# chaoting-sun/GCT-Plus

Measured on AMD Instinct MI355X. Metric: SMILES/sec training step (vaetf, seq_len=80, d_model=512), higher is better.
Workload: dtype f32

## Files before the change

### gct_plus_amd/csrc/norm.hip

```cpp
#include "common.h"

namespace {

constexpr int MAXC = 8;

template <int NC>
__global__ __launch_bounds__(256) void norm_fwd_kernel(const float* __restrict__ x,
                                                       const float* __restrict__ alpha,
                                                       const float* __restrict__ bias, float* y,
                                                       float* mean_out, float* rstd_out,
                                                       int64_t rows, int d, float eps) {
  const int lane = threadIdx.x & 63, wave = threadIdx.x >> 6;
  const int64_t nwaves = (int64_t)gridDim.x * 4;
  float4 a[NC], b[NC];
#pragma unroll
  for (int c = 0; c < NC; ++c) {
    const int col = c * 256 + lane * 4;
    if (col < d) {
      a[c] = *reinterpret_cast<const float4*>(alpha + col);
      b[c] = *reinterpret_cast<const float4*>(bias + col);
    }
  }
  for (int64_t row = (int64_t)blockIdx.x * 4 + wave; row < rows; row += nwaves) {
    const float* xr = x + row * d;
    float4 v[NC];
    float s = 0.f;
#pragma unroll
    for (int c = 0; c < NC; ++c) {
      const int col = c * 256 + lane * 4;
      v[c] = make_float4(0.f, 0.f, 0.f, 0.f);
      if (col < d) {
        v[c] = *reinterpret_cast<const float4*>(xr + col);
        s += (v[c].x + v[c].y) + (v[c].z + v[c].w);
      }
    }
    const float mean = gct_wave_sum(s) / (float)d;
    float ss = 0.f;
#pragma unroll
    for (int c = 0; c < NC; ++c) {
      const int col = c * 256 + lane * 4;
      if (col < d) {
        v[c].x -= mean; v[c].y -= mean; v[c].z -= mean; v[c].w -= mean;
        ss += (v[c].x * v[c].x + v[c].y * v[c].y) + (v[c].z * v[c].z + v[c].w * v[c].w);
      }
    }
    const float var = gct_wave_sum(ss) / (float)(d - 1);
    const float rstd = 1.0f / (sqrtf(var) + eps);
    if (lane == 0) {
      mean_out[row] = mean;
      rstd_out[row] = rstd;
    }
    float* yr = y + row * d;
#pragma unroll
    for (int c = 0; c < NC; ++c) {
      const int col = c * 256 + lane * 4;
      if (col < d) {
        float4 o;
        o.x = a[c].x * (v[c].x * rstd) + b[c].x;
        o.y = a[c].y * (v[c].y * rstd) + b[c].y;
        o.z = a[c].z * (v[c].z * rstd) + b[c].z;
        o.w = a[c].w * (v[c].w * rstd) + b[c].w;
        *reinterpret_cast<float4*>(yr + col) = o;
      }
    }
  }
}

template <int NC>
__global__ __launch_bounds__(256) void norm_bwd_kernel(const float* __restrict__ dy,
                                                       const float* __restrict__ x,
                                                       const float* __restrict__ alpha,
                                                       const float* __restrict__ mean_in,
                                                       const float* __restrict__ rstd_in,
                                                       const float* __restrict__ dres, float* dx,
                                                       float* partial, int64_t rows, int d,
                                                       float eps, const int32_t* __restrict__ qmap,
                                                       int64_t src_rows, float* dropo, uint32_t thr, float dscale,
                                                       GctRng rng) {
  const int lane = threadIdx.x & 63, wave = threadIdx.x >> 6;
  const int64_t nwaves = (int64_t)gridDim.x * 4;
  float4 a[NC], pa[NC], pb[NC];
#pragma unroll
  for (int c = 0; c < NC; ++c) {
    const int col = c * 256 + lane * 4;
    a[c] = make_float4(0.f, 0.f, 0.f, 0.f);
    if (col < d) a[c] = *reinterpret_cast<const float4*>(alpha + col);
    pa[c] = make_float4(0.f, 0.f, 0.f, 0.f);
    pb[c] = make_float4(0.f, 0.f, 0.f, 0.f);
  }
  const int64_t nquads = (rows + 3) >> 2;
  for (int64_t quad = (int64_t)blockIdx.x * 4 + wave; quad < nquads; quad += nwaves) {
   uint4 db[NC][2];
   if (dropo) {
     const int64_t oq = qmap ? (int64_t)qmap[quad] : quad;
#pragma unroll
     for (int c = 0; c < NC; ++c) {
       const int col = c * 256 + lane * 4;
       db[c][0] = gct_drop_bits(rng, (uint32_t)(oq < 0 ? 0 : oq), (uint32_t)col);
       db[c][1] = gct_drop_bits(rng, (uint32_t)(oq < 0 ? 0 : oq), (uint32_t)col + 2);
     }
   }
   for (int e4 = 0; e4 < 4; ++e4) {
    const int64_t row = quad * 4 + e4;
    if (row >= rows) break;
    int64_t srow = row;
    if (qmap) {
      const int q = qmap[row >> 2];
      if (src_rows > 0) srow = (int64_t)q * 4 + (row & 3);
      if (q < 0 || (src_rows > 0 && srow >= src_rows)) {
        float* dr0 = dx + row * d;
#pragma unroll
        for (int c = 0; c < NC; ++c) {
          const int col = c * 256 + lane * 4;
          if (col < d) {
            *reinterpret_cast<float4*>(dr0 + col) = make_float4(0.f, 0.f, 0.f, 0.f);
            if (dropo) *reinterpret_cast<float4*>(dropo + row * d + col) = make_float4(0.f, 0.f, 0.f, 0.f);
          }
        }
        continue;
      }
    }
    const float mean = mean_in[srow], r = rstd_in[srow];
    const float* xr = x + srow * d;
    const float* gr = dy + row * d;
    float4 cx[NC], g[NC];
    float s1 = 0.f, s2 = 0.f;
#pragma unroll
    for (int c = 0; c < NC; ++c) {
      const int col = c * 256 + lane * 4;
      cx[c] = make_float4(0.f, 0.f, 0.f, 0.f);
      g[c] = cx[c];
      if (col < d) {
        float4 xv = *reinterpret_cast<const float4*>(xr + col);
        const float4 dv = *reinterpret_cast<const float4*>(gr + col);
        xv.x -= mean; xv.y -= mean; xv.z -= mean; xv.w -= mean;
        cx[c] = xv;
        pa[c].x += dv.x * xv.x * r; pa[c].y += dv.y * xv.y * r;
        pa[c].z += dv.z * xv.z * r; pa[c].w += dv.w * xv.w * r;
        pb[c].x += dv.x; pb[c].y += dv.y; pb[c].z += dv.z; pb[c].w += dv.w;
        g[c] = make_float4(dv.x * a[c].x, dv.y * a[c].y, dv.z * a[c].z, dv.w * a[c].w);
        s1 += (g[c].x + g[c].y) + (g[c].z + g[c].w);
        s2 += (g[c].x * xv.x + g[c].y * xv.y) + (g[c].z * xv.z + g[c].w * xv.w);
      }
    }
    s1 = gct_wave_sum(s1) / (float)d;
    s2 = gct_wave_sum(s2);
    const float sigma = 1.0f / r - eps;
    const float k2 = sigma > 0.f ? s2 * r * r / (sigma * (float)(d - 1)) : 0.f;
    float* dr = dx + row * d;
#pragma unroll
    for (int c = 0; c < NC; ++c) {
      const int col = c * 256 + lane * 4;
      if (col < d) {
        float4 o;
        o.x = r * (g[c].x - s1) - cx[c].x * k2;
        o.y = r * (g[c].y - s1) - cx[c].y * k2;
        o.z = r * (g[c].z - s1) - cx[c].z * k2;
        o.w = r * (g[c].w - s1) - cx[c].w * k2;
        if (dres) {
          const float4 e = *reinterpret_cast<const float4*>(dres + row * d + col);
          o.x += e.x; o.y += e.y; o.z += e.z; o.w += e.w;
        }
        *reinterpret_cast<float4*>(dr + col) = o;
        if (dropo) {
          const int e = e4;
          const uint4 b0 = db[c][0], b1 = db[c][1];
          float4 m;
// ... 9 lines not shown
  }
  __shared__ float4 comb[4][64];
#pragma unroll
  for (int c = 0; c < NC; ++c) {
    const int col = c * 256 + lane * 4;
    for (int which = 0; which < 2; ++which) {
      __syncthreads();
      comb[wave][lane] = which == 0 ? pa[c] : pb[c];
      __syncthreads();
      if (wave == 0 && col < d) {
        float4 t = comb[0][lane];
        for (int w = 1; w < 4; ++w) {
          t.x += comb[w][lane].x; t.y += comb[w][lane].y;
          t.z += comb[w][lane].z; t.w += comb[w][lane].w;
        }
        *reinterpret_cast<float4*>(partial + ((int64_t)blockIdx.x * 2 + which) * d + col) = t;
      }
    }
  }
}

inline int norm_blocks(int64_t rows) {
  int64_t b = (rows + 3) / 4;
  if (b > 1024) b = 1024;
  if (b < 1) b = 1;
  return (int)b;
}

}

int gct_reduce_slabs_seg(const float* slabs, int nslab, int64_t stride, float* d0, float* d1,
                         float* d2, int64_t nper_elems, int64_t n, hipStream_t st);

#define NORM_DISPATCH(KERNEL, ...)                                                      \
  do {                                                                                  \
    const int nc = (d + 255) / 256;                                                     \
    if (nc <= 1) hipLaunchKernelGGL((KERNEL<1>), grid, dim3(256), 0, st, __VA_ARGS__);  \
    else if (nc <= 2) hipLaunchKernelGGL((KERNEL<2>), grid, dim3(256), 0, st, __VA_ARGS__); \
    else if (nc <= 4) hipLaunchKernelGGL((KERNEL<4>), grid, dim3(256), 0, st, __VA_ARGS__); \
    else hipLaunchKernelGGL((KERNEL<8>), grid, dim3(256), 0, st, __VA_ARGS__);          \
  } while (0)

extern "C" int gct_norm_fwd(const float* x, const float* alpha, const float* bias, float* y,
                            float* mean, float* rstd, int64_t rows, int d, float eps,
                            void* stream) {
  GCT_CHECK_ARG(x && alpha && bias && y && mean && rstd, "norm_fwd: null pointer");
  GCT_CHECK_ARG(rows >= 0 && d >= 4 && d % 4 == 0 && d <= 256 * MAXC, "norm_fwd: d=%d unsupported", d);
  GCT_CHECK_ARG(gct_aligned16(x) && gct_aligned16(y) && gct_aligned16(alpha) && gct_aligned16(bias),
                "norm_fwd: pointers must be 16-B aligned");
  if (rows == 0) return GCT_OK;
  hipStream_t st = (hipStream_t)stream;
  dim3 grid((unsigned)((rows + 3) / 4 > 8192 ? 8192 : (rows + 3) / 4));
  NORM_DISPATCH(norm_fwd_kernel, x, alpha, bias, y, mean, rstd, rows, d, eps);
  GCT_LAUNCH_CHECK("norm_fwd");
  return GCT_OK;
}

extern "C" int gct_norm_bwd(const float* dy, const float* x, const float* alpha, const float* mean,
                            const float* rstd, const float* dres, float* dx, float* dalpha,
                            float* dbias, float* ws, int64_t rows, int d, float eps,
                            const int32_t* quad_map, int64_t src_rows, float* drop_out, float p, uint64_t seed,
                            uint32_t site, void* stream) {
  GCT_CHECK_ARG(dy && x && alpha && mean && rstd && dx && dalpha && dbias && ws,
                "norm_bwd: null pointer");
  GCT_CHECK_ARG(!drop_out || (gct_aligned16(drop_out) && p >= 0.f && p < 1.f), "norm_bwd: bad dropout output");
  GCT_CHECK_ARG(!quad_map || (rows % 4 == 0 && src_rows >= 0), "norm_bwd: compacted rows come in quads");
  GCT_CHECK_ARG(rows >= 0 && d >= 4 && d % 4 == 0 && d <= 256 * MAXC, "norm_bwd: d=%d unsupported", d);
  GCT_CHECK_ARG(gct_aligned16(dy) && gct_aligned16(x) && gct_aligned16(dx) && gct_aligned16(alpha) &&
                    gct_aligned16(ws) && (!dres || gct_aligned16(dres)),
                "norm_bwd: pointers must be 16-B aligned");
  hipStream_t st = (hipStream_t)stream;
  const int nblk = norm_blocks(rows);
  dim3 grid((unsigned)nblk);
  NORM_DISPATCH(norm_bwd_kernel, dy, x, alpha, mean, rstd, dres, dx, ws, rows, d, eps, quad_map, src_rows, drop_out,
                gct_drop_threshold(p), 1.0f / (1.0f - p), gct_rng_make(seed, site));
  GCT_LAUNCH_CHECK("norm_bwd");
  return gct_reduce_slabs_seg(ws, nblk, (int64_t)2 * d, dalpha, dbias, nullptr, d, (int64_t)2 * d, st);
}
```

### gct_plus_amd/engine.py

```python
from __future__ import annotations

import math
import os
from typing import List, NamedTuple, Optional

import torch
from torch.autograd.function import once_differentiable

from . import ops
from .flat import HANDED_SLOTS

_SEED = {"base": None, "ctr": 0}

COMPACT_BWD = os.environ.get("GCT_COMPACT_BWD", "1") != "0"
COMPACT_MAX_FRACTION = 0.85
COMPACT_KV = os.environ.get("GCT_COMPACT_KV", "1") != "0"
COMPACT_FWD = os.environ.get("GCT_COMPACT_FWD", "1") != "0"
COMPACT_ENC_KV = os.environ.get("GCT_COMPACT_ENC_KV", "1") != "0"
KV_FOLD = True


GRAD_NOTIFY = None


# ... 210 lines not shown
class EncoderSaved(NamedTuple):
    src: torch.Tensor
    econds: Optional[torch.Tensor]
    site_pe: int
    layers: List[EncLayerSaved]
    x_last: torch.Tensor
    mean: torch.Tensor
    rstd: torch.Tensor
    B: int
    L: int


class DecoderSaved(NamedTuple):
    trg: torch.Tensor
    z2: torch.Tensor
    dconds: Optional[torch.Tensor]
    site_pe: int
    layers: List[DecLayerSaved]
    x_last: torch.Tensor
    mean: torch.Tensor
    rstd: torch.Tensor
    B: int
    T: int
    Le: int
    Lk: int
    c2d: bool
    c2l: bool
    trg_mask_u8: Optional[torch.Tensor]
    keys: object
    live: object
    fold: object = None


def mha_fwd(run: Run, m, xq, xkv, B, Lq, Lk, mask_u8, resid, want_probs=False, keys=None, live=None, fold=None):
    d, H = m.d_model, m.h
    dk = d // H
    self_attn = xkv is xq
    Mq = xq.shape[0]
    self_split = self_attn and keys is not None and live is None and not want_probs
    if self_split:
        xkv = keys.gather(xq)
    if self_attn and not self_split:
        qkv = _empty(Mq, 3 * d, xq)
        ops.linear_fwd(xq, [m.q_linear.weight, m.k_linear.weight, m.v_linear.weight],
                       [m.q_linear.bias, m.k_linear.bias, m.v_linear.bias],
                       [qkv, qkv[:, d:], qkv[:, 2 * d:]], 3 * d)
        q, k, v, ldq, ldkv = qkv, qkv[:, d:], qkv[:, 2 * d:], 3 * d, 3 * d
        qb, kvb = qkv, None
        if live is not None:
            keys = live
    else:
        qb = _empty(Mq, d, xq)
        ops.linear_fwd(xq, [m.q_linear.weight], [m.q_linear.bias], [qb], d)
        kvb = _empty(B * Lk, 2 * d, xkv) if keys is None else keys.empty(2 * d)
        if fold is not None:
            fold[0].fwd(fold[1], xkv, [kvb, kvb[:, d:]], 2 * d)
        else:
            ops.linear_fwd(xkv, [m.k_linear.weight, m.v_linear.weight],
                           [m.k_linear.bias, m.v_linear.bias], [kvb, kvb[:, d:]], 2 * d)
        q, k, v, ldq, ldkv = qb, kvb, kvb[:, d:], d, 2 * d
    site_p = run.site()
    o, lse, probs = ops.attn_fwd(q, k, v, ldq, ldkv, ldkv, mask_u8, B, H, Lq, Lk, dk, run.p,
                                 run.seed, site_p, want_probs=want_probs, keys=keys, live=live)
    y = _empty(Mq, d, xq)
    site_o = run.site()
    if resid is not None:
        ops.linear_fwd(o, [m.out.weight], [m.out.bias], [y], d, epi=ops.EPI_DROP_RESID,
                       resid=resid, p=run.p, seed=run.seed, site=site_o, live=live)
    else:
        ops.linear_fwd(o, [m.out.weight], [m.out.bias], [y], d)
    saved = MhaSaved(xq, xkv, qb, kvb, o, lse, mask_u8, B, Lq, Lk, site_p, site_o, resid is not None,
                     None if (self_attn and live is not None) else keys, self_split)
    return y, saved, probs


def mha_bwd(run: Run, m, sv: MhaSaved, dy, G: GradSink, dxq_out, depi_q, dxkv_out=None,
            depi_kv=ops.DEPI_STORE, live=None, gdrop=None, fold=None):
    B, Lq, Lk, keys = sv.B, sv.Lq, sv.Lk, sv.keys
    d, H = m.d_model, m.h
    dk = d // H
    Mq, Mk = B * Lq, sv.xkv.shape[0]
    kt = run.kt
    new = lambda cols: _empty(Mq, cols, dy)
    if live is not None:
        Mq, kt = live.Mc, None
        new = live.empty_zero_gaps
        o_in, xq_in = (sv.o, sv.xq) if live.fwd else (live.gather(sv.o), live.gather(sv.xq))
    else:
        o_in, xq_in = sv.o, sv.xq
    if gdrop is not None:
        g = gdrop
    else:
        g = ops.dropout_bwd(dy, run.p, run.seed, sv.site_o, live=live) if (sv.fused and run.p > 0) else dy
    do = _empty(Mq, d, dy) if live is None else live.empty(d)
    ops.linear_bwd([g], d, o_in, [m.out.weight], [G(m.out.weight)], [G(m.out.bias)], do, kt=kt, M=Mq)
    if sv.kvb is None:
        dqkv = new(3 * d)
        fwdc = live is not None and live.fwd
        ops.attn_bwd(sv.qb, sv.qb[:, d:], sv.qb[:, 2 * d:], 3 * d, 3 * d, 3 * d, sv.mask_u8, sv.o, do, sv.lse, dqkv,
                     dqkv[:, d:], dqkv[:, 2 * d:], 3 * d, 3 * d, 3 * d, B, H, Lq, Lk, dk, run.p,
                     run.seed, sv.site_p, live=live, kv_compact=live is not None and not fwdc,
                     keys=live if fwdc else None)
        segs = [dqkv, dqkv[:, d:], dqkv[:, 2 * d:]]
        ops.linear_bwd(segs, 3 * d, xq_in, [m.q_linear.weight, m.k_linear.weight, m.v_linear.weight],
                       [G(m.q_linear.weight), G(m.k_linear.weight), G(m.v_linear.weight)],
                       [G(m.q_linear.bias), G(m.k_linear.bias), G(m.v_linear.bias)], dxq_out, depi=depi_q, kt=kt, M=Mq)
    else:
        dq = new(d)
        if keys is None:
            dkv = _empty(Mk, 2 * d, dy)
        else:
            dkv = keys.empty_zero_gaps(2 * d)
        ops.attn_bwd(sv.qb, sv.kvb, sv.kvb[:, d:], d, 2 * d, 2 * d, sv.mask_u8, sv.o, do, sv.lse, dq, dkv, dkv[:, d:],
                     d, 2 * d, 2 * d, B, H, Lq, Lk, dk, run.p, run.seed, sv.site_p, live=live, keys=keys)
        ops.linear_bwd([dq], d, xq_in, [m.q_linear.weight], [G(m.q_linear.weight)], [G(m.q_linear.bias)], dxq_out,
                       depi=depi_q, kt=kt, M=Mq)
        if fold is not None:
            fold[0].bwd(fold[1], [dkv, dkv[:, d:]], 2 * d, sv.xkv, dxkv_out, depi_kv, Mk)
            return
        kv_w = [m.k_linear.weight, m.v_linear.weight]
        kv_g = ([G(m.k_linear.weight), G(m.v_linear.weight)], [G(m.k_linear.bias), G(m.v_linear.bias)])
        if sv.self_split:
            dxk = keys.empty(d)
            ops.linear_bwd([dkv, dkv[:, d:]], 2 * d, sv.xkv, kv_w, *kv_g, dxk, M=Mk)
            keys.scatter_add(dxk, dxq_out)
        elif dxkv_out is not None:
            ops.linear_bwd([dkv, dkv[:, d:]], 2 * d, sv.xkv, kv_w, *kv_g, dxkv_out, depi=depi_kv, M=Mk)
        else:
            ops.linear_wgrad([dkv, dkv[:, d:]], 2 * d, sv.xkv, *kv_g)


def ffn_fwd(run: Run, ff, x, resid, live=None):
    M, d = x.shape
    dff = ff.linear_1.weight.shape[0]
    gelu_d = _empty(M, dff, x)
    hdn = _empty(M, dff, x)
    site_h = run.site()
    ops.linear_fwd(x, [ff.linear_1.weight], [ff.linear_1.bias], [hdn], dff, epi=ops.EPI_GELU_DROP_SAVE,
                   pre=gelu_d, p=run.p, seed=run.seed, site=site_h, live=live)
    y = _empty(M, d, x)
    site_o = run.site()
    if resid is not None:
        ops.linear_fwd(hdn, [ff.linear_2.weight], [ff.linear_2.bias], [y], d,
                       epi=ops.EPI_DROP_RESID, resid=resid, p=run.p, seed=run.seed, site=site_o, live=live)
    else:
        ops.linear_fwd(hdn, [ff.linear_2.weight], [ff.linear_2.bias], [y], d)
    return y, FfnSaved(x, gelu_d, hdn, site_h, site_o, resid is not None)


def ffn_bwd(run: Run, ff, sv: FfnSaved, dy, G: GradSink, dx_out, depi, live=None, gdrop=None):
    x, gelu_d, hdn = sv.x, sv.gelu_d, sv.hdn
    M, d = x.shape
    dff = gelu_d.shape[1]
    kt = run.kt
    if live is not None:
        M, kt = live.Mc, None
        if not live.fwd:
            x, hdn = live.gather(x), live.gather(hdn)
    if gdrop is not None:
        g = gdrop
    else:
        g = ops.dropout_bwd(dy, run.p, run.seed, sv.site_o, live=live) if (sv.fused and run.p > 0) else dy
    dpre = _empty(M, dff, dy) if live is None else live.empty(dff)
    ops.linear_bwd([g], d, hdn, [ff.linear_2.weight], [G(ff.linear_2.weight)], [G(ff.linear_2.bias)], dpre,
                   depi=ops.DEPI_MUL_SAVED, pre=gelu_d, p=run.p, seed=run.seed, site=sv.site_h, kt=kt, live=live,
                   pre_full=live is not None and not live.fwd, M=M)
    ops.linear_bwd([dpre], dff, x, [ff.linear_1.weight], [G(ff.linear_1.weight)], [G(ff.linear_1.bias)], dx_out,
                   depi=depi, kt=kt, M=M)


def enc_layer_fwd(run: Run, layer, x_in, B, L, mask_u8, want_probs=False, keys=None):
    n1, m1, r1 = ops.norm_fwd(x_in, layer.norm_1.alpha, layer.norm_1.bias, layer.norm_1.eps)
    a, sv_a, probs = mha_fwd(run, layer.attn, n1, n1, B, L, L, mask_u8, n1, want_probs, keys=keys)
    n2, m2, r2 = ops.norm_fwd(a, layer.norm_2.alpha, layer.norm_2.bias, layer.norm_2.eps)
    out, sv_f = ffn_fwd(run, layer.ff, n2, n2)
    return out, EncLayerSaved(x_in, m1, r1, sv_a, a, m2, r2, sv_f), probs


def _mha_drop(run: Run, sv: MhaSaved, buf):
    return (buf, run.p, run.seed, sv.site_o) if (buf is not None and sv.fused and run.p > 0) else None


def _ffn_drop(run: Run, sv: Optional[FfnSaved], buf):
    return (buf, run.p, run.seed, sv.site_o) if (buf is not None and sv is not None and sv.fused and run.p > 0) else None


def enc_layer_bwd(run: Run, layer, sv: EncLayerSaved, g, G: GradSink, gd=None, gdbuf=None, below=None):
    with ops.deferred_reductions():
        ffn_bwd(run, layer.ff, sv.ffn, g, G, g, ops.DEPI_ACCUM, gdrop=gd)
        dr = _mha_drop(run, sv.attn, gdbuf)
        ops.norm_bwd(g, sv.a, layer.norm_2.alpha, sv.m2, sv.r2, G(layer.norm_2.alpha), G(layer.norm_2.bias),
                     out=g, eps=layer.norm_2.eps, drop=dr)
        mha_bwd(run, layer.attn, sv.attn, g, G, g, ops.DEPI_ACCUM, gdrop=None if dr is None else gdbuf)
        dr = _ffn_drop(run, below, gdbuf)
        ops.norm_bwd(g, sv.x_in, layer.norm_1.alpha, sv.m1, sv.r1, G(layer.norm_1.alpha), G(layer.norm_1.bias),
                     out=g, eps=layer.norm_1.eps, drop=dr)
    _grads_done(layer, G)
    return g, (None if dr is None else gdbuf)


def dec_layer_fwd(run: Run, layer, x, e, B, T, Lk, src_mask_u8, trg_mask_u8, want_probs=False, keys=None, live=None,
                  fold=None):
    x2, m1, r1 = ops.norm_fwd(x, layer.norm_1.alpha, layer.norm_1.bias, layer.norm_1.eps)
    xa, sa1, p1 = mha_fwd(run, layer.attn_1, x2, x2, B, T, T, trg_mask_u8, x, want_probs, live=live)
    x2, m2, r2 = ops.norm_fwd(xa, layer.norm_2.alpha, layer.norm_2.bias, layer.norm_2.eps)
    xb, sa2, p2 = mha_fwd(run, layer.attn_2, x2, e, B, T, Lk, src_mask_u8, xa, want_probs, keys=keys, live=live,
                          fold=fold)
    x2, m3, r3 = ops.norm_fwd(xb, layer.norm_3.alpha, layer.norm_3.bias, layer.norm_3.eps)
    xc, sf = ffn_fwd(run, layer.ff, x2, xb, live=live)
    return xc, DecLayerSaved(x, m1, r1, sa1, xa, m2, r2, sa2, xb, m3, r3, sf), p1, p2


def dec_layer_bwd(run: Run, layer, sv: DecLayerSaved, g, de, first_de, G: GradSink, live=None, gd=None, gdbuf=None,
                  below=None, fold=None):
    t = torch.empty_like(g) if live is None else live.empty(g.shape[1])
    with ops.deferred_reductions():
        ffn_bwd(run, layer.ff, sv.ffn, g, G, t, ops.DEPI_STORE, live=live, gdrop=gd)
        dr = _mha_drop(run, sv.attn_2, gdbuf)
        ops.norm_bwd(t, sv.xb, layer.norm_3.alpha, sv.m3, sv.r3, G(layer.norm_3.alpha), G(layer.norm_3.bias),
                     dres=g, out=g, eps=layer.norm_3.eps, live=live, drop=dr)
        mha_bwd(run, layer.attn_2, sv.attn_2, g, G, t, ops.DEPI_STORE, de,
                ops.DEPI_STORE if first_de else ops.DEPI_ACCUM, live=live, gdrop=None if dr is None else gdbuf,
                fold=fold)
        dr = _mha_drop(run, sv.attn_1, gdbuf)
        ops.norm_bwd(t, sv.xa, layer.norm_2.alpha, sv.m2, sv.r2, G(layer.norm_2.alpha), G(layer.norm_2.bias),
                     dres=g, out=g, eps=layer.norm_2.eps, live=live, drop=dr)
        mha_bwd(run, layer.attn_1, sv.attn_1, g, G, t, ops.DEPI_STORE, live=live, gdrop=None if dr is None else gdbuf)
        dr = _ffn_drop(run, below, gdbuf)
        ops.norm_bwd(t, sv.x, layer.norm_1.alpha, sv.m1, sv.r1, G(layer.norm_1.alpha), G(layer.norm_1.bias),
# ... 608 lines not shown
```

### gct_plus_amd/ops.py

```python
from __future__ import annotations

import contextlib
import math
import os
import threading
import weakref
from typing import List, Optional, Sequence

import torch

from . import _lib
from ._lib import check

EPI_BIAS, EPI_GELU_DROP, EPI_DROP_RESID, EPI_GELU_DROP_SAVE = 0, 1, 2, 3
DEPI_STORE, DEPI_ACCUM, DEPI_GELU_BWD, DEPI_MUL_SAVED = 0, 1, 2, 3


def _L():
    return _lib.load()


_raw_stream, _cur_dev = torch._C._cuda_getCurrentRawStream, torch._C._cuda_getDevice


# ... 98 lines not shown

    def __exit__(self, et, ev, tb):
        if self.mine:
            _DEFER_TL.d["on"] = False
            _DEFER_TL.d["want"] = max(_DEFER_TL.d["want"], _DEFER_TL.d["demand"])
            rc = _L().gct_reduce_defer_end(_st())
            if et is None:
                check(rc, "gct_reduce_defer_end")
        return False


_WS_NEED = {}


def _ws_need(fn: str, a: int, b: int, c: int) -> int:
    key = (fn, a, b, c)
    v = _WS_NEED.get(key)
    if v is None:
        v = _WS_NEED[key] = int(getattr(_L(), fn)(a, b, c))
    return v


def norm_fwd(x2d, alpha, bias, eps=1e-6, out=None):
    _chk(x2d, "norm_fwd.x")
    rows, d = x2d.shape
    y = torch.empty_like(x2d) if out is None else out
    mean = torch.empty(rows, dtype=torch.float32, device=x2d.device)
    rstd = torch.empty(rows, dtype=torch.float32, device=x2d.device)
    check(_L().gct_norm_fwd(_p(x2d), _p(alpha), _p(bias), _p(y), _p(mean), _p(rstd), rows, d, eps,
                            _st()), "gct_norm_fwd")
    return y, mean, rstd


def norm_bwd(dy, x2d, alpha, mean, rstd, dalpha, dbias, dres=None, out=None, eps=1e-6, live=None, drop=None):
    src_rows, d = x2d.shape
    rows = src_rows if live is None else live.Mc
    if live is not None and live.fwd:
        src_rows = 0
    dx = (torch.empty_like(x2d) if live is None else live.empty(d)) if out is None else out
    _wait_pending(out)
    if drop is not None:
        _wait_pending(drop[0])
    ws = kept_workspace(_L().gct_rowred_ws_bytes(rows, 2 * d), x2d.device)
    check(_L().gct_norm_bwd(_p(dy), _p(x2d), _p(alpha), _p(mean), _p(rstd), _p(dres), _p(dx),
                            _p(dalpha), _p(dbias), _p(ws), rows, d, eps,
                            None if live is None else _p(live.quad_list), src_rows,
                            None if drop is None else _p(drop[0]), 0.0 if drop is None else drop[1],
                            0 if drop is None else drop[2], 0 if drop is None else drop[3], _st()), "gct_norm_bwd")
    return dx


def embed_pe_fwd(tok, table, cond, pe2d, n_c, scale, p, seed, site, d=None):
    _chk(tok, "embed.tok", torch.int64)
    B, S = tok.shape
    if table is not None:
        vocab, d = table.shape
    else:
        vocab = 1
    out = torch.empty(B * (S + n_c), d, dtype=torch.float32, device=pe2d.device)
    check(_L().gct_embed_pe_fwd(_p(tok), _p(table), _p(cond), _p(pe2d), _p(out), B, S, n_c, d, vocab,
                                scale, p, seed, site, _st()), "gct_embed_pe_fwd")
    return out


def embed_pe_bwd(dout, tok, dtable, dcond, n_c, scale, p, seed, site, d=None):
    B, S = tok.shape
    if dtable is not None:
        vocab, d = dtable.shape
    else:
        vocab = 1
    ws = kept_workspace(_L().gct_embed_ws_bytes(B, S, d, vocab), dout.device)
    check(_L().gct_embed_pe_bwd(_p(dout), _p(tok), _p(dtable), _p(dcond), _p(ws), B, S, n_c, d, vocab,
                                scale, p, seed, site, _st()), "gct_embed_pe_bwd")


PROFILE = None
PROFILE_KINDS = None


class _Timed:
    def __init__(self, kind, flops, nbytes=0):
# ... 200 lines not shown


def assert_no_skipped_row_gradients():
    n = int(skipped_row_gradients().item())
    if n:
        skipped_row_gradients().zero_()
        raise _lib.GctError(_SKIPPED_MSG.format(n))


def skipped_row_gradients():
    dev = torch.cuda.current_device()
    t = _SKIPPED.get(dev)
    if t is None:
        t = _SKIPPED[dev] = torch.zeros(1, dtype=torch.int32, device=torch.device("cuda", dev))
    return t


class LiveRows:
    SLACK = 256
    fwd = False

    def __init__(self, g2d, B, T, mask_u8, lists=True):
        _chk(g2d, "g2d")
        dev = g2d.device
        M = B * T
        assert g2d.shape[0] == M
        nt, nq = (M + 31) // 32, (M + 3) // 4
        i32 = lambda n: torch.empty(max(n, 1), dtype=torch.int32, device=dev)
        self.B, self.T, self.M, self.dev = B, T, M, dev
        self.live = torch.empty(max(M, 1), dtype=torch.uint8, device=dev)
        self.n_b, self.info = i32(B), i32(8)
        self.cstart = i32(B) if lists else None
        self.quad_list = i32(nq + 32) if lists else None
        qrank = i32(nq) if lists else None
        self.tile_list, self.tile_count = i32(nt), i32(1)
        flags = torch.empty(max(nt, 1), dtype=torch.uint8, device=dev)
        if mask_u8 is None:
            sb = sq = 0
        else:
            _chk(mask_u8, "live_rows.mask", torch.uint8)
            sb, sq = _mask_strides(mask_u8, B, T, T)
        check(_L().gct_live_rows(_p(g2d), g2d.stride(0), B, T, g2d.shape[1], _p(mask_u8), sb, sq, _p(self.live),
                                 _p(self.n_b), _p(self.info), _p(self.cstart), _p(self.quad_list), _p(qrank),
                                 _p(self.tile_list), _p(self.tile_count), _p(flags), _st()), "gct_live_rows")
        self.kt = (self.tile_list, self.tile_count)
        self._host = None
        self.Mc = None

    @classmethod
    def from_rows(cls, rows_u8, B, T, mask_u8):
        _chk(rows_u8, "live_rows.rows", torch.uint8)
        return cls(rows_u8.reshape(B * T, 1).to(torch.float32), B, T, mask_u8)

    def _fill_host(self, v):
        self._host = dict(n_live=v[0], violations=v[1], nonprefix=v[2], tiles=v[3], padded=v[4], quads=v[5], empty=v[6])
        self.Mc = v[4]

    def host(self):
        if self._host is None:
            PendingReadBack(self).finish()
        return self._host

    def scatter_add(self, src2d, dst2d):
        cols = src2d.shape[1]
        check(_L().gct_scatter_add_quads(_p(src2d), src2d.stride(0), _p(self.quad_list), self.Mc, cols, _p(dst2d),
                                         dst2d.stride(0), self.M, _st()), "gct_scatter_add_quads")
        return dst2d

    def check_grad(self, g2d):
        check(_L().gct_dead_rows_nonzero(_p(g2d), g2d.stride(0), self.M, g2d.shape[1], _p(self.live),
                                         _p(skipped_row_gradients()), _st()), "gct_dead_rows_nonzero")

    def empty(self, cols):
        return torch.empty(self.Mc + self.SLACK, cols, dtype=torch.float32, device=self.dev)[:self.Mc]

    def empty_zero_gaps(self, cols):
# ... 35 lines not shown
            self.host.copy_(dev, non_blocking=True)
            self.ev = torch.cuda.Event()
            self.ev.record()

    def finish(self):
        if self.host is None:
            return
        import time
        t0 = time.perf_counter()
        self.ev.synchronize()
        HOST_BLOCKED_S[0] += time.perf_counter() - t0
        v = self.host.tolist()
        self.host = None
        for i, o in enumerate(self.objs):
            if o._host is None:
                o._fill_host(v[8 * i:8 * i + 8])
        if v[-1] != 0:
            skipped_row_gradients().zero_()
            raise _lib.GctError(_SKIPPED_MSG.format(v[-1]))


class KeyRows(LiveRows):

    def __init__(self, mask_u8, B, Lk):
        _chk(mask_u8, "key_rows.mask", torch.uint8)
        dev = mask_u8.device
        M = B * Lk
        nq = (M + 3) // 4
        i32 = lambda n: torch.empty(max(n, 1), dtype=torch.int32, device=dev)
        self.B, self.T, self.M, self.dev = B, Lk, M, dev
        self.live = torch.empty(max(M, 1), dtype=torch.uint8, device=dev)
        self.n_b, self.info = i32(B), i32(8)
        self.cstart, self.quad_list = i32(B), i32(nq + 32)
        qrank = i32(nq)
        check(_L().gct_key_rows(_p(mask_u8), Lk, B, Lk, _p(self.live), _p(self.n_b), _p(self.info), _p(self.cstart),
                                _p(self.quad_list), _p(qrank), _st()), "gct_key_rows")
        self._host = None
        self.Mc = None



def linear_wgrad(dys: Sequence[torch.Tensor], lddy: int, x2d, dws: Sequence[torch.Tensor],
                 dbs: Sequence[Optional[torch.Tensor]], kt=None):
    M, K = x2d.shape
    nper = dws[0].shape[0]
    nseg = len(dws)
    d = _seg3(dys)
    dw = _seg3(dws)
    db = _seg3(dbs)

    def launch():
        ws = kept_workspace(_ws_need("gct_wgrad_ws_bytes", M, nseg * nper, K), x2d.device)
        with _Timed("gemm_wgrad+bias+reduce", 2.0 * M * K * nper * nseg):
            check(_L().gct_linear_wgrad(d[0], d[1], d[2], lddy, M, nseg, nper, _p(x2d), x2d.stride(0),
                                        K, dw[0], dw[1], dw[2], K, db[0], db[1], db[2], _p(ws),
                                        _p(kt[0]) if kt else None, _p(kt[1]) if kt else None, _st()),
                  "gct_linear_wgrad")

    if not SIDE_ENABLED or torch.cuda.is_current_stream_capturing():
        launch()
        return
    main = torch.cuda.current_stream()
    side = _side_stream(x2d.device)
    ready = torch.cuda.Event()
    ready.record(main)
    side.wait_event(ready)
    with torch.cuda.stream(side):
        launch()
        done = torch.cuda.Event()
# ... 841 lines not shown
```

### include/gctplus_hip.h

```cpp
#ifndef GCTPLUS_HIP_H
#define GCTPLUS_HIP_H

#include <stdint.h>

#ifdef __cplusplus
extern "C" {
#endif

#define GCT_OK 0
#define GCT_ERR_ARG (-1)
#define GCT_ERR_HIP (-2)

#define GCT_ABI_VERSION 33

int gct_version(void);
const char* gct_last_error(void);

int64_t gct_wgrad_ws_bytes(int64_t M, int64_t Ntot, int64_t K);
int64_t gct_rowred_ws_bytes(int64_t rows, int64_t cols);

int gct_norm_fwd(const float* x, const float* alpha, const float* bias, float* y,
                 float* mean, float* rstd, int64_t rows, int d, float eps, void* stream);
int gct_norm_bwd(const float* dy, const float* x, const float* alpha, const float* mean,
                 const float* rstd, const float* dres, float* dx, float* dalpha, float* dbias,
                 float* ws, int64_t rows, int d, float eps, const int32_t* quad_map, int64_t src_rows,
                 float* drop_out, float p, uint64_t seed, uint32_t site, void* stream);

int gct_embed_pe_fwd(const int64_t* tok, const float* table, const float* cond, const float* pe,
                     float* out, int B, int S, int n_c, int d, int vocab, float scale, float p,
                     uint64_t seed, uint32_t site, void* stream);
int64_t gct_embed_ws_bytes(int B, int S, int d, int vocab);
int gct_embed_pe_bwd(const float* dout, const int64_t* tok, float* dtable, float* dcond,
                     float* ws, int B, int S, int n_c, int d, int vocab, float scale, float p,
                     uint64_t seed, uint32_t site, void* stream);

#define GCT_EPI_BIAS 0
#define GCT_EPI_GELU_DROP 1
#define GCT_EPI_DROP_RESID 2
#define GCT_EPI_GELU_DROP_SAVE 3
int gct_linear_fwd(const float* x, int64_t ldx, int64_t M, int K,
                   const float* w0, const float* w1, const float* w2, int64_t ldw,
                   const uint16_t* wp0, int64_t plane_stride,
                   const float* b0, const float* b1, const float* b2,
                   int nseg, int nper, float* y0, float* y1, float* y2, int64_t ldy,
                   int epi, const float* resid, float* pre, float p, uint64_t seed, uint32_t site,
                   float* ws, int64_t ws_bytes, const int32_t* quad_map, void* stream);
int64_t gct_linear_fwd_ws_bytes(int64_t M, int K, int Ntot);

#define GCT_DEPI_STORE 0
#define GCT_DEPI_ACCUM 1
#define GCT_DEPI_GELU_BWD 2
#define GCT_DEPI_MUL_SAVED 3
int gct_linear_dgrad(const float* dy0, const float* dy1, const float* dy2, int64_t lddy,
                     int64_t M, int nseg, int nper,
                     const float* w0, const float* w1, const float* w2, int64_t ldw,
                     const uint16_t* wp0, int64_t plane_stride, int K,
                     float* dx, int64_t lddx, int depi, const float* pre, float p, uint64_t seed,
                     uint32_t site, float* ws, int64_t ws_bytes, const int32_t* quad_map, int64_t pre_rows,
                     void* stream);
// ... 298 lines not shown
```

Before: 11770.

## Fuse key-row gather into norm forward and scatter-add into norm backward

The encoder's first layer norm now also writes the compacted live-key rows straight from its forward kernel, so the separate gather launch for self-attention keys/values is no longer needed. In backward, the compact key gradient is added inside the norm backward kernel rather than through a separate scatter-add into the residual gradient. This removes two extra kernel launches and a full read-modify-write pass over the activations per encoder layer. In exchange the norm kernels gain per-quad rank lookups and a tail pass that zero-fills padding rows, and the engine now has more plumbing through the compaction metadata.

```diff
diff --git a/gct_plus_amd/csrc/norm.hip b/gct_plus_amd/csrc/norm.hip
--- a/gct_plus_amd/csrc/norm.hip
+++ b/gct_plus_amd/csrc/norm.hip
@@ -4,12 +4,26 @@
 
 constexpr int MAXC = 8;
 
-template <int NC>
+__device__ __forceinline__ int64_t norm_compact_quad(const int32_t* __restrict__ qrank, const uint8_t* __restrict__ live,
+                                                     int64_t rows, int64_t cquads, int64_t q) {
+  const int64_t qs = __builtin_amdgcn_readfirstlane((int)q);
+  const int64_t rk = qrank[qs];
+  uint32_t f = 0;
+  if (qs * 4 + 4 <= rows) f = *reinterpret_cast<const uint32_t*>(live + qs * 4);
+  else
+    for (int64_t r = qs * 4; r < rows; ++r) f |= live[r];
+  return (f != 0 && rk < cquads) ? rk : -1;
+}
+
+template <int NC, bool COPY>
 __global__ __launch_bounds__(256) void norm_fwd_kernel(const float* __restrict__ x,
                                                        const float* __restrict__ alpha,
                                                        const float* __restrict__ bias, float* y,
                                                        float* mean_out, float* rstd_out,
-                                                       int64_t rows, int d, float eps) {
+                                                       int64_t rows, int d, float eps,
+                                                       const int32_t* __restrict__ qlist,
+                                                       const int32_t* __restrict__ qrank,
+                                                       const uint8_t* __restrict__ live, int64_t cquads, float* yc) {
   const int lane = threadIdx.x & 63, wave = threadIdx.x >> 6;
   const int64_t nwaves = (int64_t)gridDim.x * 4;
   float4 a[NC], b[NC];
@@ -21,8 +35,13 @@
       b[c] = *reinterpret_cast<const float4*>(bias + col);
     }
   }
+  int64_t cq_next = -1;
+  if (COPY && (int64_t)blockIdx.x * 4 + wave < rows)
+    cq_next = norm_compact_quad(qrank, live, rows, cquads, ((int64_t)blockIdx.x * 4 + wave) >> 2);
   for (int64_t row = (int64_t)blockIdx.x * 4 + wave; row < rows; row += nwaves) {
     const float* xr = x + row * d;
+    const int64_t crow = cq_next >= 0 ? cq_next * 4 + (row & 3) : -1;
+    if (COPY && row + nwaves < rows) cq_next = norm_compact_quad(qrank, live, rows, cquads, (row + nwaves) >> 2);
     float4 v[NC];
     float s = 0.f;
 #pragma unroll
@@ -61,12 +80,27 @@
         o.z = a[c].z * (v[c].z * rstd) + b[c].z;
         o.w = a[c].w * (v[c].w * rstd) + b[c].w;
         *reinterpret_cast<float4*>(yr + col) = o;
-      }
-    }
-  }
-}
-
-template <int NC>
+        if (COPY && crow >= 0) *reinterpret_cast<float4*>(yc + crow * d + col) = o;
+      }
+    }
+  }
+  if (COPY) {
+    const float4 z = make_float4(0.f, 0.f, 0.f, 0.f);
+    for (int64_t cq = (int64_t)blockIdx.x * 4 + wave; cq < cquads; cq += nwaves) {
+      const int64_t q = qlist[cq];
+      for (int e = 0; e < 4; ++e)
+        if (q < 0 || q * 4 + e >= rows) {
+#pragma unroll
+          for (int c = 0; c < NC; ++c) {
+            const int col = c * 256 + lane * 4;
+            if (col < d) *reinterpret_cast<float4*>(yc + (cq * 4 + e) * d + col) = z;
+          }
+        }
+    }
+  }
+}
+
+template <int NC, bool ADD>
 __global__ __launch_bounds__(256) void norm_bwd_kernel(const float* __restrict__ dy,
                                                        const float* __restrict__ x,
                                                        const float* __restrict__ alpha,
@@ -76,7 +110,9 @@
                                                        float* partial, int64_t rows, int d,
                                                        float eps, const int32_t* __restrict__ qmap,
                                                        int64_t src_rows, float* dropo, uint32_t thr, float dscale,
-                                                       GctRng rng) {
+                                                       GctRng rng, const float* __restrict__ addc,
+                                                       const int32_t* __restrict__ aqrank,
+                                                       const uint8_t* __restrict__ alive, int64_t acquads) {
   const int lane = threadIdx.x & 63, wave = threadIdx.x >> 6;
   const int64_t nwaves = (int64_t)gridDim.x * 4;
   float4 a[NC], pa[NC], pb[NC];
@@ -89,6 +125,9 @@
     pb[c] = make_float4(0.f, 0.f, 0.f, 0.f);
   }
   const int64_t nquads = (rows + 3) >> 2;
+  int64_t aq_next = -1;
+  if (ADD && (int64_t)blockIdx.x * 4 + wave < nquads)
+    aq_next = norm_compact_quad(aqrank, alive, rows, acquads, (int64_t)blockIdx.x * 4 + wave);
   for (int64_t quad = (int64_t)blockIdx.x * 4 + wave; quad < nquads; quad += nwaves) {
    uint4 db[NC][2];
    if (dropo) {
@@ -100,6 +139,8 @@
        db[c][1] = gct_drop_bits(rng, (uint32_t)(oq < 0 ? 0 : oq), (uint32_t)col + 2);
      }
    }
+   const int64_t arow0 = aq_next >= 0 ? aq_next * 4 : -1;
+   if (ADD && quad + nwaves < nquads) aq_next = norm_compact_quad(aqrank, alive, rows, acquads, quad + nwaves);
    for (int e4 = 0; e4 < 4; ++e4) {
     const int64_t row = quad * 4 + e4;
     if (row >= rows) break;
@@ -132,7 +173,11 @@
       g[c] = cx[c];
       if (col < d) {
         float4 xv = *reinterpret_cast<const float4*>(xr + col);
-        const float4 dv = *reinterpret_cast<const float4*>(gr + col);
+        float4 dv = *reinterpret_cast<const float4*>(gr + col);
+        if (ADD && arow0 >= 0) {
+          const float4 av = *reinterpret_cast<const float4*>(addc + (arow0 + e4) * d + col);
+          dv.x += av.x; dv.y += av.y; dv.z += av.z; dv.w += av.w;
+        }
         xv.x -= mean; xv.y -= mean; xv.z -= mean; xv.w -= mean;
         cx[c] = xv;
         pa[c].x += dv.x * xv.x * r; pa[c].y += dv.y * xv.y * r;
@@ -208,35 +253,58 @@
 int gct_reduce_slabs_seg(const float* slabs, int nslab, int64_t stride, float* d0, float* d1,
                          float* d2, int64_t nper_elems, int64_t n, hipStream_t st);
 
-#define NORM_DISPATCH(KERNEL, ...)                                                      \
-  do {                                                                                  \
-    const int nc = (d + 255) / 256;                                                     \
-    if (nc <= 1) hipLaunchKernelGGL((KERNEL<1>), grid, dim3(256), 0, st, __VA_ARGS__);  \
-    else if (nc <= 2) hipLaunchKernelGGL((KERNEL<2>), grid, dim3(256), 0, st, __VA_ARGS__); \
-    else if (nc <= 4) hipLaunchKernelGGL((KERNEL<4>), grid, dim3(256), 0, st, __VA_ARGS__); \
-    else hipLaunchKernelGGL((KERNEL<8>), grid, dim3(256), 0, st, __VA_ARGS__);          \
+#define NORM_DISPATCH(KERNEL, FLAG, ...)                                                      \
+  do {                                                                                        \
+    const int nc = (d + 255) / 256;                                                           \
+    if (nc <= 1) hipLaunchKernelGGL((KERNEL<1, FLAG>), grid, dim3(256), 0, st, __VA_ARGS__);  \
+    else if (nc <= 2) hipLaunchKernelGGL((KERNEL<2, FLAG>), grid, dim3(256), 0, st, __VA_ARGS__); \
+    else if (nc <= 4) hipLaunchKernelGGL((KERNEL<4, FLAG>), grid, dim3(256), 0, st, __VA_ARGS__); \
+    else hipLaunchKernelGGL((KERNEL<8, FLAG>), grid, dim3(256), 0, st, __VA_ARGS__);          \
   } while (0)
 
-extern "C" int gct_norm_fwd(const float* x, const float* alpha, const float* bias, float* y,
-                            float* mean, float* rstd, int64_t rows, int d, float eps,
-                            void* stream) {
+extern "C" int gct_norm_fwd_rows(const float* x, const float* alpha, const float* bias, float* y, float* mean,
+                                 float* rstd, int64_t rows, int d, float eps, const int32_t* quad_list,
+                                 const int32_t* quad_rank, const uint8_t* live, int64_t crows, float* yc, void* stream) {
   GCT_CHECK_ARG(x && alpha && bias && y && mean && rstd, "norm_fwd: null pointer");
   GCT_CHECK_ARG(rows >= 0 && d >= 4 && d % 4 == 0 && d <= 256 * MAXC, "norm_fwd: d=%d unsupported", d);
   GCT_CHECK_ARG(gct_aligned16(x) && gct_aligned16(y) && gct_aligned16(alpha) && gct_aligned16(bias),
                 "norm_fwd: pointers must be 16-B aligned");
+  GCT_CHECK_ARG((quad_list == nullptr) == (quad_rank == nullptr) && (quad_list == nullptr) == (yc == nullptr) &&
+                    (quad_list == nullptr) == (live == nullptr),
+                "norm_fwd: quad_list / quad_rank / live / yc go together");
+  GCT_CHECK_ARG(!quad_list || (crows >= 0 && crows % 4 == 0 && gct_aligned16(yc) &&
+                               (reinterpret_cast<uintptr_t>(live) & 3u) == 0),
+                "norm_fwd: the compact copy is whole quads of 16-B aligned rows, live is 4-B aligned");
+  hipStream_t st = (hipStream_t)stream;
+  if (quad_list) {
+    if (rows == 0 && crows == 0) return GCT_OK;
+    int64_t work = (rows + 3) / 4 > crows / 16 ? (rows + 3) / 4 : crows / 16;
+    dim3 grid((unsigned)(work > 8192 ? 8192 : (work < 1 ? 1 : work)));
+    NORM_DISPATCH(norm_fwd_kernel, true, x, alpha, bias, y, mean, rstd, rows, d, eps, quad_list, quad_rank, live, crows / 4,
+                  yc);
+    GCT_LAUNCH_CHECK("norm_fwd_rows");
+    return GCT_OK;
+  }
   if (rows == 0) return GCT_OK;
-  hipStream_t st = (hipStream_t)stream;
   dim3 grid((unsigned)((rows + 3) / 4 > 8192 ? 8192 : (rows + 3) / 4));
-  NORM_DISPATCH(norm_fwd_kernel, x, alpha, bias, y, mean, rstd, rows, d, eps);
+  NORM_DISPATCH(norm_fwd_kernel, false, x, alpha, bias, y, mean, rstd, rows, d, eps, (const int32_t*)nullptr,
+                (const int32_t*)nullptr, (const uint8_t*)nullptr, (int64_t)0, (float*)nullptr);
   GCT_LAUNCH_CHECK("norm_fwd");
   return GCT_OK;
 }
 
-extern "C" int gct_norm_bwd(const float* dy, const float* x, const float* alpha, const float* mean,
-                            const float* rstd, const float* dres, float* dx, float* dalpha,
-                            float* dbias, float* ws, int64_t rows, int d, float eps,
-                            const int32_t* quad_map, int64_t src_rows, float* drop_out, float p, uint64_t seed,
-                            uint32_t site, void* stream) {
+extern "C" int gct_norm_fwd(const float* x, const float* alpha, const float* bias, float* y,
+                            float* mean, float* rstd, int64_t rows, int d, float eps,
+                            void* stream) {
+  return gct_norm_fwd_rows(x, alpha, bias, y, mean, rstd, rows, d, eps, nullptr, nullptr, nullptr, 0, nullptr, stream);
+}
+
+extern "C" int gct_norm_bwd_rows(const float* dy, const float* x, const float* alpha, const float* mean,
+                                 const float* rstd, const float* dres, float* dx, float* dalpha, float* dbias, float* ws,
+                                 int64_t rows, int d, float eps, const int32_t* quad_map, int64_t src_rows,
+                                 float* drop_out, float p, uint64_t seed, uint32_t site, const float* add,
+                                 const int32_t* add_quad_rank, const uint8_t* add_live, int64_t add_rows,
+                                 void* stream) {
   GCT_CHECK_ARG(dy && x && alpha && mean && rstd && dx && dalpha && dbias && ws,
                 "norm_bwd: null pointer");
   GCT_CHECK_ARG(!drop_out || (gct_aligned16(drop_out) && p >= 0.f && p < 1.f), "norm_bwd: bad dropout output");
@@ -245,11 +313,32 @@
   GCT_CHECK_ARG(gct_aligned16(dy) && gct_aligned16(x) && gct_aligned16(dx) && gct_aligned16(alpha) &&
                     gct_aligned16(ws) && (!dres || gct_aligned16(dres)),
                 "norm_bwd: pointers must be 16-B aligned");
+  GCT_CHECK_ARG((add == nullptr) == (add_quad_rank == nullptr) && (add == nullptr) == (add_live == nullptr),
+                "norm_bwd: add / add_quad_rank / add_live go together");
+  GCT_CHECK_ARG(!add || (!quad_map && add_rows >= 0 && add_rows % 4 == 0 && gct_aligned16(add) &&
+                         (reinterpret_cast<uintptr_t>(add_live) & 3u) == 0),
+                "norm_bwd: the compact addend is whole quads of 16-B aligned rows, add_live is 4-B aligned, and dy is not "
+                "compacted itself");
   hipStream_t st = (hipStream_t)stream;
   const int nblk = norm_blocks(rows);
   dim3 grid((unsigned)nblk);
-  NORM_DISPATCH(norm_bwd_kernel, dy, x, alpha, mean, rstd, dres, dx, ws, rows, d, eps, quad_map, src_rows, drop_out,
-                gct_drop_threshold(p), 1.0f / (1.0f - p), gct_rng_make(seed, site));
+  if (add)
+    NORM_DISPATCH(norm_bwd_kernel, true, dy, x, alpha, mean, rstd, dres, dx, ws, rows, d, eps, quad_map, src_rows, drop_out,
+                  gct_drop_threshold(p), 1.0f / (1.0f - p), gct_rng_make(seed, site), add, add_quad_rank, add_live,
+                  add_rows / 4);
+  else
+    NORM_DISPATCH(norm_bwd_kernel, false, dy, x, alpha, mean, rstd, dres, dx, ws, rows, d, eps, quad_map, src_rows,
+                  drop_out, gct_drop_threshold(p), 1.0f / (1.0f - p), gct_rng_make(seed, site), (const float*)nullptr,
+                  (const int32_t*)nullptr, (const uint8_t*)nullptr, (int64_t)0);
   GCT_LAUNCH_CHECK("norm_bwd");
   return gct_reduce_slabs_seg(ws, nblk, (int64_t)2 * d, dalpha, dbias, nullptr, d, (int64_t)2 * d, st);
 }
+
+extern "C" int gct_norm_bwd(const float* dy, const float* x, const float* alpha, const float* mean,
+                            const float* rstd, const float* dres, float* dx, float* dalpha,
+                            float* dbias, float* ws, int64_t rows, int d, float eps,
+                            const int32_t* quad_map, int64_t src_rows, float* drop_out, float p, uint64_t seed,
+                            uint32_t site, void* stream) {
+  return gct_norm_bwd_rows(dy, x, alpha, mean, rstd, dres, dx, dalpha, dbias, ws, rows, d, eps, quad_map, src_rows,
+                           drop_out, p, seed, site, nullptr, nullptr, nullptr, 0, stream);
+}
diff --git a/gct_plus_amd/engine.py b/gct_plus_amd/engine.py
--- a/gct_plus_amd/engine.py
+++ b/gct_plus_amd/engine.py
@@ -266,14 +266,19 @@
     fold: object = None
 
 
-def mha_fwd(run: Run, m, xq, xkv, B, Lq, Lk, mask_u8, resid, want_probs=False, keys=None, live=None, fold=None):
+def mha_self_split(keys, live, want_probs):
+    return keys is not None and live is None and not want_probs
+
+
+def mha_fwd(run: Run, m, xq, xkv, B, Lq, Lk, mask_u8, resid, want_probs=False, keys=None, live=None, fold=None,
+            xq_rows=None):
     d, H = m.d_model, m.h
     dk = d // H
     self_attn = xkv is xq
     Mq = xq.shape[0]
-    self_split = self_attn and keys is not None and live is None and not want_probs
+    self_split = self_attn and mha_self_split(keys, live, want_probs)
     if self_split:
-        xkv = keys.gather(xq)
+        xkv = keys.gather(xq) if xq_rows is None else xq_rows
     if self_attn and not self_split:
         qkv = _empty(Mq, 3 * d, xq)
         ops.linear_fwd(xq, [m.q_linear.weight, m.k_linear.weight, m.v_linear.weight],
@@ -309,7 +314,7 @@
 
 
 def mha_bwd(run: Run, m, sv: MhaSaved, dy, G: GradSink, dxq_out, depi_q, dxkv_out=None,
-            depi_kv=ops.DEPI_STORE, live=None, gdrop=None, fold=None):
+            depi_kv=ops.DEPI_STORE, live=None, gdrop=None, fold=None, add_kv=True):
     B, Lq, Lk, keys = sv.B, sv.Lq, sv.Lk, sv.keys
     d, H = m.d_model, m.h
     dk = d // H
@@ -357,6 +362,8 @@
         if sv.self_split:
             dxk = keys.empty(d)
             ops.linear_bwd([dkv, dkv[:, d:]], 2 * d, sv.xkv, kv_w, *kv_g, dxk, M=Mk)
+            if not add_kv:
+                return dxk
             keys.scatter_add(dxk, dxq_out)
         elif dxkv_out is not None:
             ops.linear_bwd([dkv, dkv[:, d:]], 2 * d, sv.xkv, kv_w, *kv_g, dxkv_out, depi=depi_kv, M=Mk)
@@ -404,8 +411,12 @@
 
 
 def enc_layer_fwd(run: Run, layer, x_in, B, L, mask_u8, want_probs=False, keys=None):
-    n1, m1, r1 = ops.norm_fwd(x_in, layer.norm_1.alpha, layer.norm_1.bias, layer.norm_1.eps)
-    a, sv_a, probs = mha_fwd(run, layer.attn, n1, n1, B, L, L, mask_u8, n1, want_probs, keys=keys)
+    n1k = None
+    if mha_self_split(keys, None, want_probs):
+        n1, m1, r1, n1k = ops.norm_fwd_rows(x_in, layer.norm_1.alpha, layer.norm_1.bias, keys, layer.norm_1.eps)
+    else:
+        n1, m1, r1 = ops.norm_fwd(x_in, layer.norm_1.alpha, layer.norm_1.bias, layer.norm_1.eps)
+    a, sv_a, probs = mha_fwd(run, layer.attn, n1, n1, B, L, L, mask_u8, n1, want_probs, keys=keys, xq_rows=n1k)
     n2, m2, r2 = ops.norm_fwd(a, layer.norm_2.alpha, layer.norm_2.bias, layer.norm_2.eps)
     out, sv_f = ffn_fwd(run, layer.ff, n2, n2)
     return out, EncLayerSaved(x_in, m1, r1, sv_a, a, m2, r2, sv_f), probs
@@ -425,10 +436,11 @@
         dr = _mha_drop(run, sv.attn, gdbuf)
         ops.norm_bwd(g, sv.a, layer.norm_2.alpha, sv.m2, sv.r2, G(layer.norm_2.alpha), G(layer.norm_2.bias),
                      out=g, eps=layer.norm_2.eps, drop=dr)
-        mha_bwd(run, layer.attn, sv.attn, g, G, g, ops.DEPI_ACCUM, gdrop=None if dr is None else gdbuf)
+        dxk = mha_bwd(run, layer.attn, sv.attn, g, G, g, ops.DEPI_ACCUM, gdrop=None if dr is None else gdbuf,
+                      add_kv=False)
         dr = _ffn_drop(run, below, gdbuf)
         ops.norm_bwd(g, sv.x_in, layer.norm_1.alpha, sv.m1, sv.r1, G(layer.norm_1.alpha), G(layer.norm_1.bias),
-                     out=g, eps=layer.norm_1.eps, drop=dr)
+                     out=g, eps=layer.norm_1.eps, drop=dr, add=None if dxk is None else (dxk, sv.attn.keys))
     _grads_done(layer, G)
     return g, (None if dr is None else gdbuf)
 
diff --git a/gct_plus_amd/ops.py b/gct_plus_amd/ops.py
--- a/gct_plus_amd/ops.py
+++ b/gct_plus_amd/ops.py
@@ -154,7 +154,21 @@
     return y, mean, rstd
 
 
-def norm_bwd(dy, x2d, alpha, mean, rstd, dalpha, dbias, dres=None, out=None, eps=1e-6, live=None, drop=None):
+def norm_fwd_rows(x2d, alpha, bias, keys, eps=1e-6):
+    _chk(x2d, "norm_fwd.x")
+    rows, d = x2d.shape
+    assert rows == keys.M, "the quad map covers other rows than x"
+    y = torch.empty_like(x2d)
+    yc = keys.empty(d)
+    mean = torch.empty(rows, dtype=torch.float32, device=x2d.device)
+    rstd = torch.empty(rows, dtype=torch.float32, device=x2d.device)
+    check(_L().gct_norm_fwd_rows(_p(x2d), _p(alpha), _p(bias), _p(y), _p(mean), _p(rstd), rows, d, eps,
+                                 _p(keys.quad_list), _p(keys.quad_rank), _p(keys.live), keys.Mc, _p(yc), _st()),
+          "gct_norm_fwd_rows")
+    return y, mean, rstd, yc
+
+
+def norm_bwd(dy, x2d, alpha, mean, rstd, dalpha, dbias, dres=None, out=None, eps=1e-6, live=None, drop=None, add=None):
     src_rows, d = x2d.shape
     rows = src_rows if live is None else live.Mc
     if live is not None and live.fwd:
@@ -164,11 +178,17 @@
     if drop is not None:
         _wait_pending(drop[0])
     ws = kept_workspace(_L().gct_rowred_ws_bytes(rows, 2 * d), x2d.device)
-    check(_L().gct_norm_bwd(_p(dy), _p(x2d), _p(alpha), _p(mean), _p(rstd), _p(dres), _p(dx),
-                            _p(dalpha), _p(dbias), _p(ws), rows, d, eps,
-                            None if live is None else _p(live.quad_list), src_rows,
-                            None if drop is None else _p(drop[0]), 0.0 if drop is None else drop[1],
-                            0 if drop is None else drop[2], 0 if drop is None else drop[3], _st()), "gct_norm_bwd")
+    args = (_p(dy), _p(x2d), _p(alpha), _p(mean), _p(rstd), _p(dres), _p(dx), _p(dalpha), _p(dbias), _p(ws), rows, d, eps,
+            None if live is None else _p(live.quad_list), src_rows,
+            None if drop is None else _p(drop[0]), 0.0 if drop is None else drop[1],
+            0 if drop is None else drop[2], 0 if drop is None else drop[3])
+    if add is None:
+        check(_L().gct_norm_bwd(*args, _st()), "gct_norm_bwd")
+    else:
+        rows_c, keys = add
+        assert live is None and keys.M == src_rows and tuple(rows_c.shape) == (keys.Mc, d) and rows_c.is_contiguous()
+        check(_L().gct_norm_bwd_rows(*args, _p(rows_c), _p(keys.quad_rank), _p(keys.live), keys.Mc, _st()),
+              "gct_norm_bwd_rows")
     return dx
 
 
@@ -435,7 +455,7 @@
         self.n_b, self.info = i32(B), i32(8)
         self.cstart = i32(B) if lists else None
         self.quad_list = i32(nq + 32) if lists else None
-        qrank = i32(nq) if lists else None
+        self.quad_rank = i32(nq) if lists else None
         self.tile_list, self.tile_count = i32(nt), i32(1)
         flags = torch.empty(max(nt, 1), dtype=torch.uint8, device=dev)
         if mask_u8 is None:
@@ -444,7 +464,7 @@
             _chk(mask_u8, "live_rows.mask", torch.uint8)
             sb, sq = _mask_strides(mask_u8, B, T, T)
         check(_L().gct_live_rows(_p(g2d), g2d.stride(0), B, T, g2d.shape[1], _p(mask_u8), sb, sq, _p(self.live),
-                                 _p(self.n_b), _p(self.info), _p(self.cstart), _p(self.quad_list), _p(qrank),
+                                 _p(self.n_b), _p(self.info), _p(self.cstart), _p(self.quad_list), _p(self.quad_rank),
                                  _p(self.tile_list), _p(self.tile_count), _p(flags), _st()), "gct_live_rows")
         self.kt = (self.tile_list, self.tile_count)
         self._host = None
@@ -546,9 +566,9 @@
         self.live = torch.empty(max(M, 1), dtype=torch.uint8, device=dev)
         self.n_b, self.info = i32(B), i32(8)
         self.cstart, self.quad_list = i32(B), i32(nq + 32)
-        qrank = i32(nq)
+        self.quad_rank = i32(nq)
         check(_L().gct_key_rows(_p(mask_u8), Lk, B, Lk, _p(self.live), _p(self.n_b), _p(self.info), _p(self.cstart),
-                                _p(self.quad_list), _p(qrank), _st()), "gct_key_rows")
+                                _p(self.quad_list), _p(self.quad_rank), _st()), "gct_key_rows")
         self._host = None
         self.Mc = None
 
diff --git a/include/gctplus_hip.h b/include/gctplus_hip.h
--- a/include/gctplus_hip.h
+++ b/include/gctplus_hip.h
@@ -25,6 +25,14 @@
                  const float* rstd, const float* dres, float* dx, float* dalpha, float* dbias,
                  float* ws, int64_t rows, int d, float eps, const int32_t* quad_map, int64_t src_rows,
                  float* drop_out, float p, uint64_t seed, uint32_t site, void* stream);
+int gct_norm_fwd_rows(const float* x, const float* alpha, const float* bias, float* y, float* mean, float* rstd,
+                      int64_t rows, int d, float eps, const int32_t* quad_list, const int32_t* quad_rank,
+                      const uint8_t* live, int64_t crows, float* yc, void* stream);
+int gct_norm_bwd_rows(const float* dy, const float* x, const float* alpha, const float* mean, const float* rstd,
+                      const float* dres, float* dx, float* dalpha, float* dbias, float* ws, int64_t rows, int d,
+                      float eps, const int32_t* quad_map, int64_t src_rows, float* drop_out, float p, uint64_t seed,
+                      uint32_t site, const float* add, const int32_t* add_quad_rank, const uint8_t* add_live,
+                      int64_t add_rows, void* stream);
 
 int gct_embed_pe_fwd(const int64_t* tok, const float* table, const float* cond, const float* pe,
                      float* out, int B, int S, int n_c, int d, int vocab, float scale, float p,
```

Result: no change. 11750, median of 2 (-0.2%).
